# microsoft/SEAL

Measured on NVIDIA B200. Metric: CKKS multiply+relinearize ciphertexts/s, higher is better.
Workload: dtype u64

## Files before the change

### seal_b200/csrc/sb_api.cu

```cuda
#include "../../include/seal_b200.h"
#include "sb_engine.cuh"
#include <random>
#include <algorithm>
#include <cctype>
#include <cstdio>
#include <cstring>
#include <new>
#include <thread>

using namespace sb;

static thread_local std::string g_last_error;

struct sb200_context
{
    std::unique_ptr<Context> c;
};
struct sb200_public_key
{
    PublicKey k;
    ~sb200_public_key()
    {
        if (k.d_key && k.ctx)
        {
            cudaSetDevice(k.ctx->device);
            cudaFree(k.d_key);
        }
    }
};
struct sb200_secret_key
{
    SecretKey k;
    ~sb200_secret_key()
    {
        if (k.d_pow && k.ctx)
        {
            cudaSetDevice(k.ctx->device);
            cudaMemset(k.d_pow, 0, k.powers * k.ctx->k * k.ctx->n * sizeof(u64));
            cudaDeviceSynchronize();
        }
        cudaFree(k.d_pow);
    }
};
struct sb200_kswitch_key
{
    KSwitchKey k;
    ~sb200_kswitch_key()
    {
        if (k.ctx)
            cudaSetDevice(k.ctx->device);
        cudaFree(k.d_key);
        cudaFree(k.d_key32);
    }
};

#define SB_TRY try {
#define SB_CATCH                                   \
    }                                              \
    catch (const std::invalid_argument &e)         \
    {                                              \
        g_last_error = e.what();                   \
        return SB200_E_INVALID_ARG;                \
    }                                              \
    catch (const std::out_of_range &e)             \
    {                                              \
        g_last_error = e.what();                   \
        return SB200_E_OUT_OF_RANGE;               \
    }                                              \
    catch (const std::logic_error &e)              \
    {                                              \
        g_last_error = e.what();                   \
        return SB200_E_LOGIC;                      \
    }                                              \
    catch (const std::bad_alloc &e)                \
    {                                              \
        g_last_error = e.what();                   \
        return SB200_E_NOMEM;                      \
    }                                              \
    catch (const std::exception &e)                \
    {                                              \
        g_last_error = e.what();                   \
        return SB200_E_CUDA;                       \
    }

#define SB_NEED(p)                                      \
    if (!(p))                                           \
    {                                                   \
        g_last_error = "null pointer: " #p;             \
        return SB200_E_POINTER;                         \
    }

extern "C" {

const char *sb200_last_error(void)
{
    return g_last_error.c_str();
}

int sb200_context_create(int scheme, size_t n, const uint64_t *coeff_modulus, size_t k, uint64_t plain_modulus, int device,
                         sb200_context **out)
{
    SB_NEED(coeff_modulus);
    SB_NEED(out);
    SB_TRY
    auto h = std::make_unique<sb200_context>();
    h->c = make_context(scheme, n, reinterpret_cast<const u64 *>(coeff_modulus), k, plain_modulus, device);
    *out = h.release();
    return SB200_OK;
    SB_CATCH
}

int sb200_context_destroy(sb200_context *ctx)
{
    SB_NEED(ctx);
    delete ctx;
    return SB200_OK;
}

int sb200_coeff_modulus_create(size_t n, const int *bit_sizes, size_t k, uint64_t *out)
{
    SB_NEED(bit_sizes);
    SB_NEED(out);
    SB_TRY
    if (n < 2 || (n & (n - 1)) || n > 131072)
        throw std::invalid_argument("poly_modulus_degree is invalid");
    for (size_t i = 0; i < k; i++)
        if (bit_sizes[i] < 2 || bit_sizes[i] > 60)
            throw std::invalid_argument("bit_sizes is invalid");
    auto v = sbh::coeff_modulus_create(n, std::vector<int>(bit_sizes, bit_sizes + k));
    for (size_t i = 0; i < k; i++)
        out[i] = v[i];
    return SB200_OK;
    SB_CATCH
}

int sb200_get_ntt_tables(const sb200_context *ctx, size_t i, uint64_t *root, uint64_t *rp_op, uint64_t *rp_quo, uint64_t *irp_op,
                         uint64_t *inv_n)
{
    SB_NEED(ctx);
    SB_TRY
    const Context &c = *ctx->c;
    if (i >= c.k)
        throw std::out_of_range("prime_index");
    const auto &t = c.tabs[i];
    if (root)
        *root = t.root;
    if (inv_n)
        *inv_n = t.inv_n.w;
    for (size_t j = 0; j < c.n; j++)
    {
        if (rp_op)
            rp_op[j] = t.root_powers[j].w;
        if (rp_quo)
            rp_quo[j] = t.root_powers[j].wq;
        if (irp_op)
            irp_op[j] = t.inv_root_powers[j].w;
    }
    return SB200_OK;
    SB_CATCH
}

int sb200_get_base_bsk(const sb200_context *ctx, size_t L, uint64_t *out, size_t capacity, size_t *count)
{
    SB_NEED(ctx);
    SB_NEED(out);
    SB_NEED(count);
    SB_TRY
    Context &c = *ctx->c;
    if (c.scheme != SB200_SCHEME_BFV)
        throw std::logic_error("BEHZ base exists for BFV contexts only");
    const auto &b = behz_host(c, L);
    if (b.nBsk > capacity)
        throw std::out_of_range("capacity");
    for (size_t i = 0; i < b.nBsk; i++)
        out[i] = b.Bsk[i];
    *count = b.nBsk;
    return SB200_OK;
    SB_CATCH
}

uint32_t sb200_galois_elt_from_step(const sb200_context *ctx, int step)
{
    if (!ctx)
        return 0;
    try
    {
        return sbh::galois_elt_from_step(ctx->c->n, step);
    }
    catch (const std::exception &e)
    {
        g_last_error = e.what();
        return 0;
    }
}

unsigned long long sb200_launch_count(const sb200_context *ctx)
{
    return ctx ? ctx->c->stats.launches : 0;
}

size_t sb200_device_bytes(const sb200_context *ctx)
{
    return ctx ? ctx->c->table_bytes + ctx->c->scratch_bytes + ctx->c->aux_bytes : 0;
}

// ... 1488 lines not shown
```

### seal_b200/csrc/sb_engine.cuh

```cuda
#pragma once
#include "sb_host.hpp"
#include "sb_ntt.cuh"
#include "sb_ksint.cuh"
#include "sb_wire.hpp"
#include <array>
#include <map>
#include <memory>
#include <mutex>
#include <string>
#include <vector>

namespace sb
{
    struct CudaError : std::runtime_error
    {
        using std::runtime_error::runtime_error;
    };
    void cuda_check(cudaError_t e, const char *what);

    struct BehzDev;

    struct SecretKey
    {
        struct Context *ctx = nullptr;
        u64 *d_pow = nullptr;
        size_t powers = 0;
    };

    struct PublicKey
    {
        struct Context *ctx = nullptr;
        u64 *d_key = nullptr;
    };

    struct KSwitchKey
    {
        struct Context *ctx = nullptr;
        u64 *d_key = nullptr;
        uint32_t *d_key32 = nullptr;
        size_t digits = 0;
    };

    struct IoArena
    {
        bool ready = false;
        cudaStream_t s_in = nullptr, s_comp = nullptr, s_out = nullptr;
        cudaEvent_t ev_in[2] = {}, ev_comp[2] = {}, ev_out[2] = {};
        u64 *buf[2][3] = {};
        size_t cap[2][3] = {};
        struct Lane
        {
            void *pin[2] = {};
            size_t cap = 0;
            cudaEvent_t ev[2] = {}, order = nullptr;
            cudaStream_t st = nullptr;
            std::mutex mu;
        } lane[2];
    };

    struct Context
    {
        int scheme = 0, device = 0, logn = 0;
        bool fast_q = true;
        size_t n = 0, k = 0;
        u64 t = 0;
        std::vector<u64> q;
        std::vector<sbh::PrimeTables> tabs;
        std::vector<u64> aux;
        std::vector<Tw *> d_fwd, d_inv;
        PrimeDev *d_primes = nullptr;
        size_t nprimes = 0;
        Tw *d_invq = nullptr;
        Tw *d_qmod = nullptr;
        u64 t_ratio = 0;
        std::vector<u64> inv_q_mod_t;
        struct DecryptLevel
        {
            void *d_consts = nullptr;
            u64 neg_inv_q_mod_t = 0, neg_inv_q_mod_g = 0, q_mod_t = 0;
        };
        std::map<size_t, DecryptLevel> decrypt_levels;
        int t_pid = -1;
        uint32_t *d_batch_inv_map = nullptr;
        struct PlainLevel
        {
            Tw *d_delta = nullptr;
            u64 q_mod_t = 0;
        };
        std::map<size_t, PlainLevel> plain_levels;
        struct CkksEncoder
        {
            bool ready = false;
            void *d_roots = nullptr, *d_inv_roots = nullptr;
            uint32_t *d_map = nullptr;
            void *d_stat = nullptr;
        } ckks;
        struct CkksLevel
        {
            int total_bits = 0;
            u64 *d_big = nullptr;
            Tw *d_invp = nullptr;
        };
        std::map<size_t, CkksLevel> ckks_levels;
        u64 *d_t_mod_q = nullptr;
        u64 t_ratio_lo = 0, t_ratio_hi = 0;
        std::vector<std::array<u64, 4>> parms_ids;
        std::map<uint32_t, uint32_t *> galois_tables;
        std::map<size_t, std::shared_ptr<BehzDev>> behz;
        void *scratch = nullptr;
        int *d_flag = nullptr;
        void *aux_buf = nullptr;
        size_t aux_bytes = 0;
        size_t scratch_used = 0, aux_used = 0;
        size_t scratch_bytes = 0, table_bytes = 0, scratch_budget = size_t(8) << 30;
        size_t ks_chunk_max = 0;
        size_t host_stage_bytes = size_t(640) << 20;
        LaunchStats stats;
        KsInt ksint;
        int ks_algo = 1;
        size_t ks_min_digits = 6;
        bool ksint_on(size_t L) const { return ksint.ready && (ks_algo == 2 || (ks_algo == 1 && L >= ks_min_digits)); }
        IoArena io;
        std::mutex mu;
        cudaEvent_t order_event = nullptr;
        cudaStream_t order_stream = nullptr;
        bool order_valid = false;

        ~Context();
        void *ensure_scratch(size_t bytes);
        void *ensure_aux(size_t bytes);
        void wipe_scratch(cudaStream_t st);
        void wipe_aux(cudaStream_t st);
        const uint32_t *galois_table(uint32_t elt);
        size_t prime_id_aux(size_t aux_index) const { return k + aux_index; }
    };

    std::unique_ptr<Context> make_context(int scheme, size_t n, const u64 *moduli, size_t k, u64 t, int device);

    void op_ntt(Context &c, bool inverse, size_t L, size_t size, size_t batch, u64 *d, cudaStream_t st);
    void op_linear(Context &c, int mode, size_t L, size_t size, size_t batch, const u64 *a, const u64 *b, u64 *out, cudaStream_t st);
    void op_multiply_plain(Context &c, size_t L, size_t size, size_t batch, const u64 *a, const u64 *plain, u64 *out, cudaStream_t st);
    void secret_key_create(Context &c, const u64 *h_sk, SecretKey &out);
    void op_decrypt(Context &c, SecretKey &sk, size_t L, size_t size, size_t batch, const u64 *ct, const u64 *h_cf, u64 *plain, cudaStream_t st);
    void op_batch_encode(Context &c, size_t batch, const u64 *values, u64 *plain, cudaStream_t st);
    void op_batch_decode(Context &c, size_t batch, const u64 *plain, u64 *values, cudaStream_t st);
    void op_plain_to_ntt(Context &c, size_t L, size_t batch, const u64 *plain, const u64 *h_cf, u64 *out, cudaStream_t st);
    void op_multiply_plain_coeff(Context &c, size_t L, size_t size, size_t batch, bool ct_ntt, const u64 *ct, const u64 *plain, u64 *out,
                                 cudaStream_t st);
    void op_add_plain_coeff(Context &c, size_t L, size_t size, size_t batch, bool subtract, const u64 *ct, const u64 *plain, const u64 *h_cf,
                            u64 *out, cudaStream_t st);
    void op_ckks_multiply(Context &c, size_t L, size_t batch, const u64 *a, const u64 *b, u64 *out3, cudaStream_t st);
    void op_bfv_multiply(Context &c, size_t L, size_t batch, const u64 *a, const u64 *b, u64 *out3, cudaStream_t st);
    void op_ckks_multiply(Context &c, size_t L, size_t s1, size_t s2, size_t batch, const u64 *a, const u64 *b, u64 *out, cudaStream_t st);
    void op_bfv_multiply(Context &c, size_t L, size_t s1, size_t s2, size_t batch, const u64 *a, const u64 *b, u64 *out, cudaStream_t st);
    void check_sizes(size_t s1, size_t s2);
    void launch_tensor_general(Context &c, const u64 *xa, long long xa_bs, const u64 *xb, long long xb_bs, u64 *out, const int *pid_tab,
                               size_t nb, size_t s1, size_t s2, size_t B, cudaStream_t st);
    void op_relinearize(Context &c, size_t L, size_t batch, const u64 *in3, const KSwitchKey &key, u64 *out2, cudaStream_t st);
    void op_multiply_relinearize(Context &c, size_t L, size_t batch, const u64 *a, const u64 *b, const KSwitchKey &key,
                                 u64 *out2, cudaStream_t st);
    void op_rescale(Context &c, size_t L, size_t polys, const u64 *in, u64 *out, cudaStream_t st);
    void op_mod_switch(Context &c, size_t L, size_t polys, const u64 *in, u64 *out, cudaStream_t st);
    void op_relinearize_sized(Context &c, size_t L, size_t size, size_t batch, const u64 *in, const KSwitchKey &key, u64 *out, cudaStream_t st);
    void op_apply_galois(Context &c, size_t L, size_t batch, const u64 *in2, uint32_t elt, const KSwitchKey &key, u64 *out2,
                         cudaStream_t st);
    size_t keyswitch_chunk(const Context &c, size_t L, size_t batch, bool fused);
    double selftest_rate(Context &c, int kind, cudaStream_t st);
    void op_expand_seeded(Context &c, size_t L, size_t B, const u64 *h_seeds, const long long *h_dst_off, u64 *d_out, cudaStream_t st);
    void op_encrypt_zero_symmetric(Context &c, const SecretKey &sk, size_t L, size_t B, const u64 *h_boot_seeds, bool save_seed, u64 *d_out,
                                   u64 *h_public_seeds, cudaStream_t st);
    void public_key_create(Context &c, const u64 *h_pk, PublicKey &out);
    void op_encrypt_zero_asymmetric(Context &c, const PublicKey &pk, size_t L, size_t B, const u64 *h_seeds, u64 *d_out, cudaStream_t st);
    void op_ckks_encode(Context &c, size_t L, size_t B, const double *values, size_t count, bool is_complex, double scale, u64 *plain,
                        cudaStream_t st);
    void op_ckks_decode(Context &c, size_t L, size_t B, const u64 *plain, double scale, double *values, cudaStream_t st);
    const sbh::BehzLevel &behz_host(Context &c, size_t L);
    bool op_residues_in_range(Context &c, size_t L, size_t rows, const u64 *d, cudaStream_t st);
}
```

### seal_b200/csrc/sb_ksint.cu

```cuda
#include "sb_engine.cuh"
#include "sb_ksint.cuh"
#include <algorithm>
#include <cstdlib>

namespace sb
{
    struct P32
    {
        uint32_t p, p2, np;
    };
    __device__ __forceinline__ P32 make_p32(uint32_t p) { return P32{ p, 2 * p, 0u - p }; }
    __device__ __forceinline__ uint32_t minsub(uint32_t x, uint32_t m) { return min(x, x - m); }
    __device__ __forceinline__ uint32_t mul32_lazy(uint32_t y, uint2 w, uint32_t np) { return y * w.x + __umulhi(y, w.y) * np; }
    __device__ __forceinline__ void ct32(uint32_t &x, uint32_t &y, uint2 w, const P32 &P)
    {
        const uint32_t u = minsub(x, P.p2), t = mul32_lazy(y, w, P.np);
        x = u + t;
        y = u - t + P.p2;
    }
    __device__ __forceinline__ void gs32(uint32_t &x, uint32_t &y, uint2 w, const P32 &P)
    {
        const uint32_t u = x + y, v = x - y + P.p2;
        x = minsub(u, P.p2);
        y = mul32_lazy(v, w, P.np);
// ... 332 lines not shown
        asm volatile("cp.async.wait_group %0;" ::"n"(D - 2) : "memory");
        fetch(dA, kA, 0);
        int J = 0;
#pragma unroll 1
        for (; J + 2 <= L; J += 2)
        {
            issue();
            asm volatile("cp.async.wait_group %0;" ::"n"(D - 2) : "memory");
            fetch(dB, kB, J + 1);
            macs(dA, kA);
            issue();
            asm volatile("cp.async.wait_group %0;" ::"n"(D - 2) : "memory");
            fetch(dA, kA, J + 2);
            macs(dB, kB);
        }
        if (J < L)
            macs(dA, kA);
        asm volatile("cp.async.wait_group 0;" ::: "memory");
        const P32 P = make_p32(prm.p[t]);
        const uint2 red = prm.red[t];
        const uint32_t mu = prm.mu[t];
#pragma unroll
        for (int i = 0; i < TB; i++)
        {
            if (b0 + i < B)
            {
                uint32_t *o = Acc + ((((static_cast<size_t>(b0 + i) * 2 + c) * (L + 1) + i0) * prm.S + t) << LOGN) + x;
#pragma unroll
                for (int r = 0; r < TC; r++)
                    if (i0 + r <= L)
                        o[(static_cast<size_t>(r) * prm.S) << LOGN] = minsub(reduce64(acc[i][r], red, mu, P), P.p2);
            }
        }
    }
    constexpr int kMacRingBytes = kMacStages * kMacTB * 512 * 4;
    template <int LOGN>
    __global__ void __launch_bounds__(512, 1) ks32_mac_tile(const uint32_t *__restrict__ Dh, const uint32_t *__restrict__ key32, uint32_t *__restrict__ Acc,
                                                             KsIntParams prm, int L, int k, int digits, int B, int Bpad)
    {
        constexpr int TB = kMacTB, TC = kMacTC, D = kMacStages;
        extern __shared__ __align__(16) uint32_t ks_tile[];
        const int warp = threadIdx.x >> 5, lane = threadIdx.x & 31;
        const int ntile = (L + TC) / TC, ny = (2 * ntile + 3) / 4;
        const int yg = blockIdx.x % ny, xt = blockIdx.x / ny, t = blockIdx.z;
        const int x = (xt << 5) + lane;
        const uint32_t *kbase = key32 + ((static_cast<size_t>(t) * digits * 2 * k) << LOGN) + x;
        const size_t kstep = static_cast<size_t>(2 * k) << LOGN;
        for (int rho = warp; rho < L * 32; rho += 16)
        {
            const int J = rho >> 5, tr = rho & 31;
            const int task = min(yg * 4 + (tr >> 3), 2 * ntile - 1), c = task / ntile, i0 = (task - c * ntile) * TC;
            cp_async4(ks_tile + ((((J << 3) + (tr >> 2)) << 5) + lane) * 4 + (tr & 3),
                      kbase + J * kstep + (static_cast<size_t>(c * k + i0 + (tr & 7)) << LOGN));
        }
        asm volatile("cp.async.commit_group;\n\tcp.async.wait_group 0;" ::: "memory");
        __syncthreads();
        const int bsub = warp & 3, icsub = warp >> 2;
        const int task = yg * 4 + icsub;
        if (task >= 2 * ntile)
            return;
        const int c = task / ntile, i0 = (task - c * ntile) * TC;
        const uint32_t *ktile = ks_tile + (((icsub * 2) << 5) + lane) * 4;
        uint32_t *ring = ks_tile + L * 1024 + threadIdx.x * 4;
        const P32 P = make_p32(prm.p[t]);
        const uint2 red = prm.red[t];
        const uint32_t mu = prm.mu[t];
        const size_t dstep = static_cast<size_t>(Bpad) << LOGN;
        for (int b0 = bsub * TB; b0 < B; b0 += 4 * TB)
        {
            const uint32_t *dp = Dh + ((static_cast<size_t>(t) * L * Bpad + b0) << LOGN) + x;
            u64 acc[TB][TC];
#pragma unroll
            for (int i = 0; i < TB; i++)
#pragma unroll
                for (int r = 0; r < TC; r++)
                    acc[i][r] = 0;
            auto issue_quad = [&](int stage, int J) {
#pragma unroll
                for (int h = 0; h < 4; h++)
                    if (J + h < L)
                    {
                        uint32_t *dst = ring + (stage + h) * (TB * 512);
#pragma unroll
                        for (int i = 0; i < TB; i++)
                            cp_async4(dst + i, dp + (i << LOGN));
                        dp += dstep;
                    }
                asm volatile("cp.async.commit_group;" ::: "memory");
            };
            static_assert(TB == 4 && TC == 8 && D == 8, "operand fetches are 16-byte reads; the ring holds two groups of four digits");
            auto pair_step = [&](int stage, const uint32_t *kt, bool both) {
                uint32_t d0[TB], k0[TC], d1[TB], k1[TC];
                const uint32_t *src = ring + stage * (TB * 512);
                const uint4 da = *reinterpret_cast<const uint4 *>(src), db = *reinterpret_cast<const uint4 *>(src + TB * 512);
                const uint4 ka = *reinterpret_cast<const uint4 *>(kt), kb = *reinterpret_cast<const uint4 *>(kt + 128);
                const uint4 kc = *reinterpret_cast<const uint4 *>(kt + 1024), kd = *reinterpret_cast<const uint4 *>(kt + 1024 + 128);
                d0[0] = da.x, d0[1] = da.y, d0[2] = da.z, d0[3] = da.w, d1[0] = db.x, d1[1] = db.y, d1[2] = db.z, d1[3] = db.w;
                k0[0] = ka.x, k0[1] = ka.y, k0[2] = ka.z, k0[3] = ka.w, k0[4] = kb.x, k0[5] = kb.y, k0[6] = kb.z, k0[7] = kb.w;
                k1[0] = kc.x, k1[1] = kc.y, k1[2] = kc.z, k1[3] = kc.w, k1[4] = kd.x, k1[5] = kd.y, k1[6] = kd.z, k1[7] = kd.w;
                if (both)
                {
#pragma unroll
                    for (int i = 0; i < TB; i++)
#pragma unroll
                        for (int r = 0; r < TC; r++)
                        {
                            asm("mad.wide.u32 %0, %1, %2, %0;" : "+l"(acc[i][r]) : "r"(d0[i]), "r"(k0[r]));
                            asm("mad.wide.u32 %0, %1, %2, %0;" : "+l"(acc[i][r]) : "r"(d1[i]), "r"(k1[r]));
                        }
                }
                else
                {
#pragma unroll
                    for (int i = 0; i < TB; i++)
#pragma unroll
                        for (int r = 0; r < TC; r++)
                            asm("mad.wide.u32 %0, %1, %2, %0;" : "+l"(acc[i][r]) : "r"(d0[i]), "r"(k0[r]));
                }
            };
            issue_quad(0, 0);
            const uint32_t *kt = ktile;
#pragma unroll 1
            for (int J0 = 0; J0 < L; J0 += D)
            {
#pragma unroll
                for (int u = 0; u < D; u += 4)
                {
                    const int J = J0 + u;
                    if (J >= L)
                        break;
                    issue_quad((u + 4) & (D - 1), J + 4);
                    asm volatile("cp.async.wait_group 1;" ::: "memory");
                    pair_step(u, kt, J + 1 < L);
                    if (J + 2 < L)
                        pair_step(u + 2, kt + 2048, J + 3 < L);
                    kt += 4096;
                }
            }
            asm volatile("cp.async.wait_group 0;" ::: "memory");
#pragma unroll
            for (int i = 0; i < TB; i++)
            {
                if (b0 + i < B)
                {
                    uint32_t *o = Acc + ((((static_cast<size_t>(b0 + i) * 2 + c) * (L + 1) + i0) * prm.S + t) << LOGN) + x;
#pragma unroll
                    for (int r = 0; r < TC; r++)
                        if (i0 + r <= L)
                            o[(static_cast<size_t>(r) * prm.S) << LOGN] = minsub(reduce64(acc[i][r], red, mu, P), P.p2);
                }
            }
        }
    }
    template <int LOGN>
    static void launch_mac(const KsIntScratch &s, const uint32_t *key32, const KsInt &d, int L, int k, int digits, int B, int nbt, int n,
                           cudaStream_t st)
    {
        const int ntile = (L + kMacTC) / kMacTC, ny = (2 * ntile + 3) / 4;
        const size_t tile_smem = static_cast<size_t>(L) * 4096 + kMacRingBytes;
        if (d.mac_tile && tile_smem <= 227 * 1024 && B >= 16)
        {
            cuda_check(cudaFuncSetAttribute(ks32_mac_tile<LOGN>, cudaFuncAttributeMaxDynamicSharedMemorySize, static_cast<int>(tile_smem)), "smem attr");
            dim3 grid(static_cast<unsigned>(ny) * static_cast<unsigned>(n / 32), 1, static_cast<unsigned>(d.prm.S));
            ks32_mac_tile<LOGN><<<grid, 512, tile_smem, st>>>(s.Dh, key32, s.Acc, d.prm, L, k, digits, B, nbt * kMacTB);
            return;
        }
        cuda_check(cudaFuncSetAttribute(ks32_mac<LOGN>, cudaFuncAttributeMaxDynamicSharedMemorySize, kMacSmem), "smem attr");
        dim3 grid(static_cast<unsigned>(nbt) * static_cast<unsigned>(ny) * static_cast<unsigned>(n / 32), 1, static_cast<unsigned>(d.prm.S));
        ks32_mac<LOGN><<<grid, 128, kMacSmem, st>>>(s.Dh, key32, s.Acc, d.prm, L, k, digits, B, nbt);
    }

    struct CrtArgs
    {
        const uint32_t *Acc;
        const u64 *punct, *neg;
        const PrimeDev *primes;
        const Tw *inv_top;
        const u64 *half_mod;
        const Tw *qtop_mod;
        u64 t = 0, t_ratio = 0;
        Tw inv_top_mod_t = { 0, 0 };
        u64 *R;
        u64 *out;
        long long o_bs, o_ps;
        BaseSrc base;
        int L, k;
        long long total;
    };
    template <int MODE, int LOGN, bool FUSE>
    __global__ void __launch_bounds__(FUSE ? 128 : 256) ks32_crt_kernel(CrtArgs A, KsIntParams prm, const uint2 *__restrict__ tw_outer)
    {
        constexpr int R = LOGN - 12, E = FUSE ? (1 << R) : 1;
        const int S = prm.S, L = A.L, k = A.k;
        int bc, j;
        if (FUSE)
            bc = blockIdx.x >> 5, j = ((blockIdx.x & 31) << 7) + threadIdx.x;
        else
        {
            const long long e = static_cast<long long>(blockIdx.x) * blockDim.x + threadIdx.x;
            if (e >= A.total)
                return;
            bc = static_cast<int>(e >> LOGN), j = static_cast<int>(e & ((1 << LOGN) - 1));
        }
        const int b = bc >> 1, c = bc & 1;
        const uint32_t *src = A.Acc + ((static_cast<size_t>(bc) * (L + 1) * S) << LOGN) + j;
        constexpr int PF = FUSE ? 1 : kKsMaxS;
        uint32_t nxt[PF];
        auto prefetch = [&]() {
            if (!FUSE)
            {
#pragma unroll
                for (int t = 0; t < kKsMaxS; t++)
                    if (t < S)
                        nxt[t] = src[static_cast<size_t>(t) << LOGN];
            }
        };
        prefetch();
        uint32_t nrow[FUSE ? E : 1];
        int rows_left = FUSE ? (L + 1) * S : 0;
        auto fetch_row = [&]() {
            if (FUSE)
            {
                if (rows_left > 0)
                {
#pragma unroll
                    for (int e = 0; e < E; e++)
                        nrow[e] = src[e << 12];
                }
                src += size_t(1) << LOGN;
                rows_left--;
            }
        };
        fetch_row();
        auto reconstruct = [&](int ki, const PrimeDev &Q, u64(&val)[E], bool more) {
            u64 a0[E], a1[E], f[E];
#pragma unroll
            for (int e = 0; e < E; e++)
                a0[e] = a1[e] = f[e] = 0;
            const u64 *punct = A.punct + ki * S;
            uint32_t cur[PF];
            if (!FUSE)
            {
#pragma unroll
                for (int t = 0; t < kKsMaxS; t++)
                    cur[t] = nxt[t];
                src += static_cast<size_t>(S) << LOGN;
                if (more)
                    prefetch();
            }
#pragma unroll
            for (int t = 0; t < kKsMaxS; t++)
            {
                if (t >= S)
                    break;
                const P32 P = make_p32(prm.p[t]);
                uint32_t a[E];
                if (FUSE)
                {
#pragma unroll
                    for (int e = 0; e < E; e++)
                        a[e] = nrow[e];
                    fetch_row();
                    const uint2 *tw = tw_outer + (t << R);
                    radix_inv<R>(a, [&](int lvl, int g) { return __ldg(tw + (1 << lvl) + g); }, P);
                }
                else
                    a[0] = cur[t];
                const uint2 c1 = prm.c1[t];
                const uint32_t c2 = prm.c2[t], ip = prm.inv60[t];
                const u64 C = __ldg(punct + t);
                const uint32_t C0 = static_cast<uint32_t>(C), C1 = static_cast<uint32_t>(C >> 32);
#pragma unroll
                for (int e = 0; e < E; e++)
                {
                    const uint32_t y = minsub(minsub(a[e] * c1.x + c2 + __umulhi(a[e], c1.y) * P.np, P.p2), P.p);
                    asm("mad.wide.u32 %0, %1, %2, %0;" : "+l"(a0[e]) : "r"(y), "r"(C0));
                    asm("mad.wide.u32 %0, %1, %2, %0;" : "+l"(a1[e]) : "r"(y), "r"(C1));
                    asm("mad.wide.u32 %0, %1, %2, %0;" : "+l"(f[e]) : "r"(y), "r"(ip));
                }
            }
            const u64 *neg = A.neg + ki * S;
#pragma unroll
            for (int e = 0; e < E; e++)
            {
                const u64 ng = __ldg(neg + static_cast<int>(f[e] >> 60));
                u64 lo = a0[e] + (a1[e] << 32), hi = (a1[e] >> 32) + (lo < a0[e]);
                lo += ng;
                hi += (lo < ng);
                val[e] = barrett_wide(lo, hi, Q);
            }
        };
        const PrimeDev T = A.primes[k - 1];
        u64 U[E], K[MODE == 3 ? E : 1];
        reconstruct(k - 1, T, U, L > 0);
#pragma unroll
        for (int e = 0; e < E; e++)
        {
            if (MODE == 3)
            {
                const u64 r = barrett64(U[e], A.t, A.t_ratio);
                K[e] = mul_shoup(r ? A.t - r : 0, A.inv_top_mod_t, A.t);
            }
            else
                U[e] = csub(U[e] + (T.q >> 1), T.q);
        }
        for (int i = 0; i < L; i++)
        {
            const PrimeDev Q = A.primes[i];
            u64 a[E];
            reconstruct(i, Q, a, i + 1 < L);
// ... 69 lines not shown
            const u64 t = csub(csub(v, P.q2), P.q);
            out[b * o_bs + c * o_ps + (static_cast<long long>(i) << logn) + idx] = csub(t + base.get(b, c, i, idx, P.q), P.q);
        }
        __device__ __forceinline__ void store8(int row, int idx0, u64 (&a)[8], const PrimeDev &P) const
        {
            const int i = row % L, bc = row / L, b = bc >> 1, c = bc & 1;
            ulonglong2 *op_ = reinterpret_cast<ulonglong2 *>(out + b * o_bs + c * o_ps + (static_cast<long long>(i) << logn) + idx0);
            const bool has_base = base.present && !(c == 1 && base.c1_zero);
            const bool base_plain = has_base && base.s.plain();
            const ulonglong2 *bp = base_plain ? reinterpret_cast<const ulonglong2 *>(base.s.row(b, i) + c * base.pstride + idx0) : nullptr;
#pragma unroll
            for (int h = 0; h < 4; h++)
            {
                u64 r0 = csub(csub(a[2 * h], P.q2), P.q), r1 = csub(csub(a[2 * h + 1], P.q2), P.q);
                if (base_plain)
                {
                    const ulonglong2 bv = bp[h];
                    r0 = csub(r0 + bv.x, P.q), r1 = csub(r1 + bv.y, P.q);
                }
                else if (has_base)
                {
                    r0 = csub(r0 + base.get(b, c, i, idx0 + 2 * h, P.q), P.q);
                    r1 = csub(r1 + base.get(b, c, i, idx0 + 2 * h + 1, P.q), P.q);
                }
                op_[h] = make_ulonglong2(r0, r1);
            }
        }
    };

    template <class T>
    static T *upload(const std::vector<T> &v, size_t &bytes)
    {
        T *d = nullptr;
        cuda_check(cudaMalloc(reinterpret_cast<void **>(&d), std::max<size_t>(1, v.size()) * sizeof(T)), "cudaMalloc(ksint table)");
        cuda_check(cudaMemcpy(d, v.data(), v.size() * sizeof(T), cudaMemcpyHostToDevice), "upload ksint table");
        bytes += v.size() * sizeof(T);
        return d;
    }

    void ksint_init(Context &c)
    {
        c.ksint.ready = false;
        if (c.logn < 12 || c.k < 2)
            return;
        const sbh::KsIntHost h = sbh::build_ksint(c.n, c.q.data(), c.k);
        if (h.S == 0 || h.S > kKsMaxS)
            return;
        KsInt &d = c.ksint;
        d.prm.S = h.S, d.prm.r = h.r, d.prm.logn = c.logn;
        for (int t = 0; t < h.S; t++)
        {
            d.prm.p[t] = h.p[t], d.prm.mu[t] = h.mu[t], d.prm.c2[t] = h.c2[t];
            d.prm.inv60[t] = static_cast<uint32_t>((u64(1) << 60) / h.p[t]);
            d.prm.red[t] = make_uint2(h.red[2 * t], h.red[2 * t + 1]);
            d.prm.c1[t] = make_uint2(h.c1[2 * t], h.c1[2 * t + 1]);
        }
        d.d_fwd_outer = reinterpret_cast<uint2 *>(upload(h.fwd_outer, c.table_bytes));
        d.d_inv_outer = reinterpret_cast<uint2 *>(upload(h.inv_outer, c.table_bytes));
        d.d_fwd_local = reinterpret_cast<uint2 *>(upload(h.fwd_local, c.table_bytes));
        d.d_inv_local = reinterpret_cast<uint2 *>(upload(h.inv_local, c.table_bytes));
        d.d_punct = upload(h.punct_mod_q, c.table_bytes);
        d.d_neg = upload(h.neg_mod_q, c.table_bytes);
        {
            std::vector<u64> hm(c.k);
            for (size_t i = 0; i < c.k; i++)
                hm[i] = (c.q[c.k - 1] >> 1) % c.q[i];
            d.d_half_mod = upload(hm, c.table_bytes);
        }
        cuda_check(cudaFuncSetAttribute(ks32_fwd_local, cudaFuncAttributeMaxDynamicSharedMemorySize, kKsLocalSmem), "smem attr");
        cuda_check(cudaFuncSetAttribute(ks32_inv_local, cudaFuncAttributeMaxDynamicSharedMemorySize, kKsLocalSmem), "smem attr");
        if (const char *e = std::getenv("SB200_KS_FUSE_CRT"))
            d.fuse_crt = std::atoi(e) != 0;
        if (const char *e = std::getenv("SB200_KS_MAC_TILE"))
            d.mac_tile = std::atoi(e) != 0;
        d.ready = true;
    }
    void ksint_free(Context &c)
    {
        KsInt &d = c.ksint;
        cudaFree(d.d_fwd_outer), cudaFree(d.d_inv_outer), cudaFree(d.d_fwd_local), cudaFree(d.d_inv_local), cudaFree(d.d_punct), cudaFree(d.d_neg), cudaFree(d.d_half_mod);
        d = KsInt{};
    }

    size_t ksint_bytes_per_ct(const Context &c, size_t L)
    {
        const size_t S = c.ksint.prm.S;
        return c.n * (std::max(S * L * 4, 2 * L * 8) + 2 * (L + 1) * S * 4);
    }
    size_t ksint_bytes_fixed(const Context &c, size_t L) { return c.n * c.ksint.prm.S * L * 4 * (kMacTB - 1); }
    KsIntScratch ksint_carve(const Context &c, size_t L, size_t B, void *base)
    {
        const size_t S = c.ksint.prm.S, Bpad = (B + kMacTB - 1) / kMacTB * kMacTB;
        KsIntScratch s;
        unsigned char *p = static_cast<unsigned char *>(base);
        s.Dh = reinterpret_cast<uint32_t *>(p);
        s.R = reinterpret_cast<u64 *>(p);
        p += c.n * std::max(S * L * 4 * Bpad, 2 * L * 8 * B);
        s.Acc = reinterpret_cast<uint32_t *>(p);
        return s;
    }

    template <bool PLAIN>
    static void launch_fwd_outer(Context &c, Src dsrc, int L, int rows, uint32_t *Dh, RowMap map, cudaStream_t st)
    {
        const KsInt &d = c.ksint;
        const unsigned grid = static_cast<unsigned>(rows) * 16u;
        switch (d.prm.r)
        {
        case 0: ks32_fwd_outer<0, PLAIN><<<grid, 256, 0, st>>>(dsrc, L, c.d_primes, d.prm, d.d_fwd_outer, Dh, map); break;
        case 1: ks32_fwd_outer<1, PLAIN><<<grid, 256, 0, st>>>(dsrc, L, c.d_primes, d.prm, d.d_fwd_outer, Dh, map); break;
        case 2: ks32_fwd_outer<2, PLAIN><<<grid, 256, 0, st>>>(dsrc, L, c.d_primes, d.prm, d.d_fwd_outer, Dh, map); break;
        case 3: ks32_fwd_outer<3, PLAIN><<<grid, 256, 0, st>>>(dsrc, L, c.d_primes, d.prm, d.d_fwd_outer, Dh, map); break;
        case 4: ks32_fwd_outer<4, PLAIN><<<grid, 256, 0, st>>>(dsrc, L, c.d_primes, d.prm, d.d_fwd_outer, Dh, map); break;
        case 5: ks32_fwd_outer<5, PLAIN><<<grid, 256, 0, st>>>(dsrc, L, c.d_primes, d.prm, d.d_fwd_outer, Dh, map); break;
        default: throw std::logic_error("unsupported transform size");
        }
    }

    static void ksint_forward(Context &c, Src dsrc, int L, int rows, uint32_t *Dh, RowMap map, cudaStream_t st)
    {
        const KsInt &d = c.ksint;
        const double n = static_cast<double>(c.n), S = d.prm.S;
        const bool plain = dsrc.perm == nullptr && dsrc.ginv == 0;
        c.stats.begin("ks32_fwd_outer", 0, rows * n * (8.0 + 4.0 * S), st, 0, 0);
        c.stats.work32(0.5 * rows * n * S * d.prm.r, 0);
        plain ? launch_fwd_outer<true>(c, dsrc, L, rows, Dh, map, st) : launch_fwd_outer<false>(c, dsrc, L, rows, Dh, map, st);
        c.stats.end(st);
        cuda_check(cudaGetLastError(), "ks32_fwd_outer");
        dim3 grid(static_cast<unsigned>((map.rows_out + kRowsPerCta - 1) / kRowsPerCta), static_cast<unsigned>(d.prm.S << d.prm.r));
        c.stats.begin("ks32_fwd_local", 0, rows * n * 8.0 * S, st, 0, 0);
        c.stats.work32(0.5 * rows * n * S * 12, 0);
        ks32_fwd_local<<<grid, 256, kKsLocalSmem, st>>>(Dh, map.rows_out, 1, map.rows_out, d.prm, d.d_fwd_local);
        c.stats.end(st);
        cuda_check(cudaGetLastError(), "ks32_fwd_local");
    }

    void ksint_prepare_key(Context &c, KSwitchKey &key, cudaStream_t st)
    {
        if (!c.ksint.ready || key.d_key32)
            return;
        const size_t rows = key.digits * 2 * c.k, words = rows * c.n, S = c.ksint.prm.S;
        cuda_check(cudaMalloc(reinterpret_cast<void **>(&key.d_key32), (S * words + 8 * c.n) * sizeof(uint32_t)), "cudaMalloc(key, auxiliary primes)");
        cuda_check(cudaMemsetAsync(key.d_key32 + S * words, 0, 8 * c.n * sizeof(uint32_t), st), "memset");
        u64 *tmp = nullptr;
        cuda_check(cudaMalloc(reinterpret_cast<void **>(&tmp), words * sizeof(u64)), "cudaMalloc(key staging)");
        const bool prof = c.stats.profiling;
        c.stats.profiling = false;
        try
        {
            cuda_check(cudaMemcpyAsync(tmp, key.d_key, words * sizeof(u64), cudaMemcpyDeviceToDevice, st), "key copy");
            op_ntt(c, true, c.k, 2, key.digits, tmp, st);
            ksint_forward(c, Src{ tmp, 0, nullptr, 0, c.logn }, static_cast<int>(rows), static_cast<int>(rows), key.d_key32,
                          RowMap{ 2, static_cast<int>(c.k), static_cast<int>(rows) }, st);
            cuda_check(cudaStreamSynchronize(st), "synchronize");
        }
        catch (...)
        {
            c.stats.profiling = prof;
            cudaFree(tmp);
            throw;
        }
        c.stats.profiling = prof;
        cuda_check(cudaFree(tmp), "cudaFree(key staging)");
    }

    template <int R>
    static void launch_inv_outer_r(uint32_t *data, unsigned grid, const KsInt &d, cudaStream_t st)
    {
        ks32_inv_outer<R><<<grid, 256, 0, st>>>(data, d.prm, d.d_inv_outer);
    }

    static void launch_inverse(Context &c, uint32_t *data, int arows, cudaStream_t st, bool outer = true);

    void ksint_core(Context &c, size_t L, size_t B, const KsIntScratch &s, Src dsrc, const KSwitchKey &key, BaseSrc base, u64 *out,
                    long long o_bs, cudaStream_t st)
    {
        const KsInt &d = c.ksint;
        if (!d.ready || !key.d_key32)
            throw std::logic_error("integer key-switching path is not initialised");
        const int Li = static_cast<int>(L), ki = static_cast<int>(c.k), Bi = static_cast<int>(B), S = d.prm.S;
        const double n = static_cast<double>(c.n);
        const int rows = Bi * Li, nic = 2 * (Li + 1), arows = Bi * nic;
        const int nbt = (Bi + kMacTB - 1) / kMacTB, Bpad = nbt * kMacTB;
        ksint_forward(c, dsrc, Li, rows, s.Dh, RowMap{ 1, Bpad, Li * Bpad }, st);
        {
            c.stats.begin("ks32_mac", 0, 4.0 * n * S * (static_cast<double>(Li) * 2 * (Li + 1) + rows + arows), st);
            c.stats.work32(0, static_cast<double>(arows) * Li * S * n);
            const int dg = static_cast<int>(key.digits), ni = static_cast<int>(c.n);
            switch (c.logn)
            {
            case 12: launch_mac<12>(s, key.d_key32, d, Li, ki, dg, Bi, nbt, ni, st); break;
            case 13: launch_mac<13>(s, key.d_key32, d, Li, ki, dg, Bi, nbt, ni, st); break;
            case 14: launch_mac<14>(s, key.d_key32, d, Li, ki, dg, Bi, nbt, ni, st); break;
            case 15: launch_mac<15>(s, key.d_key32, d, Li, ki, dg, Bi, nbt, ni, st); break;
            case 16: launch_mac<16>(s, key.d_key32, d, Li, ki, dg, Bi, nbt, ni, st); break;
            case 17: launch_mac<17>(s, key.d_key32, d, Li, ki, dg, Bi, nbt, ni, st); break;
            default: throw std::logic_error("unsupported transform size");
            }
            c.stats.end(st);
            cuda_check(cudaGetLastError(), "ks32_mac");
        }
        const bool fuse_crt = d.fuse_crt && d.prm.r >= 1 && d.prm.r <= 4;
        launch_inverse(c, s.Acc, arows, st, !fuse_crt);
        const long long o_ps = static_cast<long long>(L) * c.n;
        if (!o_bs)
            o_bs = 2 * o_ps;
        {
            CrtArgs A{};
            A.Acc = s.Acc, A.punct = d.d_punct, A.neg = d.d_neg, A.primes = c.d_primes;
            A.inv_top = c.d_invq + (c.k - 1) * c.k;
            A.half_mod = d.d_half_mod;
            A.R = s.R, A.out = out, A.o_bs = o_bs, A.o_ps = o_ps, A.base = base, A.L = Li, A.k = ki;
            A.total = static_cast<long long>(B) * 2 * c.n;
            c.stats.begin("ks32_crt", 0, n * B * 2 * (4.0 * S * (L + 1) + 8.0 * L), st);
            if (fuse_crt)
                c.stats.work32(0.5 * arows * S * n * d.prm.r, 0);
            if (c.scheme == 3)
            {
                A.qtop_mod = c.d_qmod + (c.k - 1) * c.k;
                A.t = c.t, A.t_ratio = c.t_ratio;
                A.inv_top_mod_t = Tw{ c.inv_q_mod_t[c.k - 1], sbh::shoup(c.inv_q_mod_t[c.k - 1], c.t) };
                launch_crt<3>(A, d, fuse_crt, B, c.logn, st);
            }
            else if (c.scheme == 1)
                launch_crt<1>(A, d, fuse_crt, B, c.logn, st);
            else
                launch_crt<0>(A, d, fuse_crt, B, c.logn, st);
            c.stats.end(st);
            cuda_check(cudaGetLastError(), "ks32_crt_kernel");
        }
        if (c.scheme != 1)
        {
            OpAddBaseFwd op{ s.R, out, o_bs, o_ps, base, c.logn, Li };
            cuda_check(launch_ntt_fwd(op, static_cast<int>(B * 2 * L), c.logn, c.d_primes, st, c.stats, "ks_result_ntt", -1, c.fast_q), "ks result ntt");
        }
    }

    static void launch_inverse(Context &c, uint32_t *data, int arows, cudaStream_t st, bool outer)
    {
        const KsInt &d = c.ksint;
        const int S = d.prm.S;
        const double n = static_cast<double>(c.n);
        dim3 grid(static_cast<unsigned>((arows + kRowsPerCta - 1) / kRowsPerCta), static_cast<unsigned>(S << d.prm.r));
        c.stats.begin("ks32_inv_local", 0, 8.0 * arows * S * n, st);
        c.stats.work32(0.5 * arows * S * n * 12, 0);
        ks32_inv_local<<<grid, 256, kKsLocalSmem, st>>>(data, arows, S, 1, d.prm, d.d_inv_local);
        c.stats.end(st);
        cuda_check(cudaGetLastError(), "ks32_inv_local");
        if (d.prm.r > 0 && outer)
        {
            const unsigned g1 = static_cast<unsigned>(arows) * S * 16u;
            c.stats.begin("ks32_inv_outer", 0, 8.0 * arows * S * n, st);
            c.stats.work32(0.5 * arows * S * n * d.prm.r, 0);
            switch (d.prm.r)
            {
            case 1: launch_inv_outer_r<1>(data, g1, d, st); break;
            case 2: launch_inv_outer_r<2>(data, g1, d, st); break;
            case 3: launch_inv_outer_r<3>(data, g1, d, st); break;
            case 4: launch_inv_outer_r<4>(data, g1, d, st); break;
            case 5: launch_inv_outer_r<5>(data, g1, d, st); break;
            default: throw std::logic_error("unsupported transform size");
            }
            c.stats.end(st);
            cuda_check(cudaGetLastError(), "ks32_inv_outer");
        }
    }

    void ksint_selftest_transform(Context &c, bool inverse, const u64 *h_rows, size_t rows, uint32_t *h_io)
    {
        if (!c.ksint.ready)
            throw std::logic_error("integer key-switching path is not available for this context");
        const size_t S = c.ksint.prm.S, out_bytes = S * rows * c.n * sizeof(uint32_t), in_bytes = rows * c.n * sizeof(u64);
        unsigned char *base = static_cast<unsigned char *>(c.ensure_scratch(out_bytes + in_bytes));
        uint32_t *d32 = reinterpret_cast<uint32_t *>(base);
        if (inverse)
        {
            cuda_check(cudaMemcpy(d32, h_io, out_bytes, cudaMemcpyHostToDevice), "upload");
            launch_inverse(c, d32, static_cast<int>(rows), nullptr);
        }
        else
        {
            u64 *d64 = reinterpret_cast<u64 *>(base + out_bytes);
            cuda_check(cudaMemcpy(d64, h_rows, in_bytes, cudaMemcpyHostToDevice), "upload");
            ksint_forward(c, Src{ d64, 0, nullptr, 0, c.logn }, static_cast<int>(rows), static_cast<int>(rows), d32,
                          RowMap{ 0, 0, static_cast<int>(rows) }, nullptr);
        }
        cuda_check(cudaMemcpy(h_io, d32, out_bytes, cudaMemcpyDeviceToHost), "download");
    }

    template <int KIND>
    __global__ void __launch_bounds__(256, 4) ks32_selftest_bfly(uint32_t *d, uint32_t p, int rounds)
    {
        __shared__ uint2 ts[256];
        const P32 P = make_p32(p);
        {
            const uint32_t w = (threadIdx.x * 2654435761u + 12345u) % p;
            ts[threadIdx.x] = make_uint2(w, static_cast<uint32_t>((static_cast<u64>(w) << 32) / p));
        }
        __syncthreads();
        uint32_t a[16];
#pragma unroll
        for (int j = 0; j < 16; j++)
            a[j] = d[(static_cast<size_t>(blockIdx.x) * 16 + j) * 256 + threadIdx.x] % p;
        const int lane = threadIdx.x & 31;
        for (int r = 0; r < rounds; r++)
        {
            const uint2 *t = ts + ((r * 7 + lane) & 127);
            auto tw = [&](int lvl, int g) { return t[(1 << lvl) - 1 + g]; };
            if (KIND == 0)
                radix_fwd<4>(a, tw, P);
            else
                radix_inv<4>(a, tw, P);
        }
#pragma unroll
        for (int j = 0; j < 16; j++)
            d[(static_cast<size_t>(blockIdx.x) * 16 + j) * 256 + threadIdx.x] = a[j];
    }
    template <int THREADS, int MINB, bool PAIRED>
    __global__ void __launch_bounds__(THREADS, MINB) ks32_selftest_mac(uint32_t *d, int rounds)
    {
        uint32_t dv[4], kv[8];
        u64 acc[4][8];
#pragma unroll
        for (int i = 0; i < 4; i++)
            dv[i] = d[(static_cast<size_t>(blockIdx.x) * 12 + i) * THREADS + threadIdx.x] >> 3;
#pragma unroll
        for (int r = 0; r < 8; r++)
            kv[r] = d[(static_cast<size_t>(blockIdx.x) * 12 + 4 + r) * THREADS + threadIdx.x] >> 3;
#pragma unroll
        for (int i = 0; i < 4; i++)
#pragma unroll
            for (int r = 0; r < 8; r++)
                acc[i][r] = 0;
        for (int q = 0; q < rounds; q++)
        {
            uint32_t d0[4], k0[8], d1[4], k1[8];
#pragma unroll
            for (int i = 0; i < 4; i++)
                d0[i] = dv[i] + q, d1[i] = dv[i] ^ q;
#pragma unroll
            for (int r = 0; r < 8; r++)
                k0[r] = kv[r] ^ q, k1[r] = kv[r] + q;
#pragma unroll
            for (int i = 0; i < 4; i++)
#pragma unroll
                for (int r = 0; r < 8; r++)
                {
                    asm("mad.wide.u32 %0, %1, %2, %0;" : "+l"(acc[i][r]) : "r"(d0[i]), "r"(k0[r]));
                    if (PAIRED)
// ... 67 lines not shown
```

Measured before the change: 2860.

## Run key-switch MAC on int8 tensor cores with byte-plane decomposed keys

Adds a tensor-core MAC kernel for the integer key-switching path. It splits the 32-bit digit and key residues into byte planes and multiplies them with u8 mma.sync, then recombines the partial sums with shifts and a modular reduction. The key is re-laid out once at key creation into a tensor-core-friendly layout and used by default when k<=32. The aim is to replace scalar 32-bit modular MACs with much higher-throughput int8 MMA work. The cost is extra key memory and about sixteen times more partial products, plus correctness risk if the accumulators overflow.

```diff
diff --git a/seal_b200/csrc/sb_api.cu b/seal_b200/csrc/sb_api.cu
--- a/seal_b200/csrc/sb_api.cu
+++ b/seal_b200/csrc/sb_api.cu
@@ -51,6 +51,7 @@
             cudaSetDevice(k.ctx->device);
         cudaFree(k.d_key);
         cudaFree(k.d_key32);
+        cudaFree(k.d_keytc);
     }
 };
 
diff --git a/seal_b200/csrc/sb_engine.cuh b/seal_b200/csrc/sb_engine.cuh
--- a/seal_b200/csrc/sb_engine.cuh
+++ b/seal_b200/csrc/sb_engine.cuh
@@ -38,6 +38,7 @@
         struct Context *ctx = nullptr;
         u64 *d_key = nullptr;
         uint32_t *d_key32 = nullptr;
+        uint32_t *d_keytc = nullptr;
         size_t digits = 0;
     };
 
diff --git a/seal_b200/csrc/sb_ksint.cu b/seal_b200/csrc/sb_ksint.cu
--- a/seal_b200/csrc/sb_ksint.cu
+++ b/seal_b200/csrc/sb_ksint.cu
@@ -508,10 +508,161 @@
             }
         }
     }
+    constexpr int kTcX = 16, kTcB = 16, kTcStage = 168 * kTcB;
+    constexpr int kTcKeyWords = 4 * 64 * 8;
+    constexpr int kTcSmem = (kTcX * kTcKeyWords + 2 * 32 * kTcB * kTcX + 2 * kTcStage) * 4;
+    static_assert(kTcSmem <= 227 * 1024, "shared memory of ks32_mac_tc");
+    __device__ __forceinline__ int tc_pos(int b, int q, int x) { return (8 * b + (q ^ (b & 4))) ^ ((x & 7) | ((x & 8) << 1)); }
+    __device__ __forceinline__ void cp_async16(uint32_t *dst_smem, const uint32_t *src, bool valid)
+    {
+        asm volatile("cp.async.cg.shared.global [%0], [%1], 16, %2;" ::"r"(smem_u32(dst_smem)), "l"(src), "r"(valid ? 16 : 0) : "memory");
+    }
+    __device__ __forceinline__ void mma_u8(uint32_t (&d)[4], const uint32_t (&a)[4], uint2 b)
+    {
+        asm("mma.sync.aligned.m16n8k32.row.col.s32.u8.u8.s32 {%0,%1,%2,%3}, {%4,%5,%6,%7}, {%8,%9}, {%0,%1,%2,%3};"
+                     : "+r"(d[0]), "+r"(d[1]), "+r"(d[2]), "+r"(d[3])
+                     : "r"(a[0]), "r"(a[1]), "r"(a[2]), "r"(a[3]), "r"(b.x), "r"(b.y));
+    }
+    __global__ void __launch_bounds__(512, 1) ks32_mac_tc(const uint32_t *__restrict__ Dh, const uint32_t *__restrict__ keytc, uint32_t *__restrict__ Acc,
+                                                          KsIntParams prm, int L, int B, int Bpad)
+    {
+        extern __shared__ __align__(16) uint32_t tc_smem[];
+        uint32_t *ks = tc_smem, *raw = ks + kTcX * kTcKeyWords, *planes = raw + 32 * kTcB * kTcX, *stage = planes + 32 * kTcB * kTcX;
+        const int tid = threadIdx.x, warp = tid >> 5, lane = tid & 31, t = blockIdx.z, x0 = blockIdx.x * kTcX, logn = prm.logn;
+        {
+            const uint32_t *src = keytc + ((static_cast<size_t>(t) << logn) + x0) * kTcKeyWords;
+            for (int i = tid; i < kTcX * kTcKeyWords / 4; i += 512)
+                cp_async16(ks + 4 * i, src + 4 * i, true);
+        }
+        auto load_raw = [&](int b0) {
+#pragma unroll
+            for (int h = 0; h < 4; h++)
+            {
+                const int i = tid + 512 * h, J = i >> 6, b = (i >> 2) & 15, xc = i & 3;
+                const bool valid = J < L && b0 + b < B;
+                const uint32_t *src = Dh + ((static_cast<size_t>(t * L + (valid ? J : 0)) * Bpad + (valid ? b0 + b : 0)) << logn) + x0 + 4 * xc;
+                cp_async16(raw + 4 * i, src, valid);
+            }
+            asm volatile("cp.async.commit_group;" ::: "memory");
+        };
+        load_raw(0);
+        asm volatile("cp.async.wait_group 0;" ::: "memory");
+        __syncthreads();
+        const P32 P = make_p32(prm.p[t]);
+        const uint2 red = prm.red[t];
+        const uint32_t mu = prm.mu[t];
+        const int g = lane >> 2, tq = lane & 3, ntc = (L + 8) / 8;
+        const uint32_t *kx = ks + warp * kTcKeyWords + 2 * tq;
+        for (int b0 = 0; b0 < B; b0 += kTcB)
+        {
+            {
+                const int x = lane & 15, b = 2 * (warp & 7) + (lane >> 4);
+#pragma unroll
+                for (int qq = 0; qq < 4; qq++)
+                {
+                    const int q = (warp >> 3) * 4 + qq;
+                    const uint32_t *r = raw + (4 * q) * (kTcB * kTcX) + b * kTcX + x;
+                    const uint32_t w0 = r[0], w1 = r[kTcB * kTcX], w2 = r[2 * kTcB * kTcX], w3 = r[3 * kTcB * kTcX];
+                    const uint32_t t0 = __byte_perm(w0, w1, 0x5140), t1 = __byte_perm(w0, w1, 0x7362);
+                    const uint32_t t2 = __byte_perm(w2, w3, 0x5140), t3 = __byte_perm(w2, w3, 0x7362);
+                    uint32_t *p = planes + x * 512 + tc_pos(b, q, x);
+                    p[0] = __byte_perm(t0, t2, 0x5410);
+                    p[128] = __byte_perm(t0, t2, 0x7632);
+                    p[256] = __byte_perm(t1, t3, 0x5410);
+                    p[384] = __byte_perm(t1, t3, 0x7632);
+                }
+            }
+            __syncthreads();
+            if (b0 + kTcB < B)
+                load_raw(b0 + kTcB);
+            uint32_t A[4][4];
+            {
+                const uint32_t *p = planes + warp * 512;
+#pragma unroll
+                for (int a = 0; a < 4; a++)
+                {
+                    A[a][0] = p[a * 128 + tc_pos(g, tq, warp)];
+                    A[a][1] = p[a * 128 + tc_pos(g + 8, tq, warp)];
+                    A[a][2] = p[a * 128 + tc_pos(g, tq + 4, warp)];
+                    A[a][3] = p[a * 128 + tc_pos(g + 8, tq + 4, warp)];
+                }
+            }
+            int j = 0;
+            for (int c = 0; c < 2; c++)
+                for (int it = 0; it < ntc; it++, j++)
+                {
+                    uint32_t C[7][4] = {};
+                    const uint32_t *kb = kx + (c * 32 + it * 8 + g) * 8;
+#pragma unroll
+                    for (int pb = 0; pb < 4; pb++)
+                    {
+                        const uint2 bf = *reinterpret_cast<const uint2 *>(kb + pb * 512);
+#pragma unroll
+                        for (int a = 0; a < 4; a++)
+                            mma_u8(C[a + pb], A[a], bf);
+                    }
+                    uint32_t *sg = stage + (j & 1) * kTcStage;
+#pragma unroll
+                    for (int h = 0; h < 2; h++)
+                    {
+                        uint32_t r[2];
+#pragma unroll
+                        for (int e = 0; e < 2; e++)
+                        {
+                            const int v = 2 * h + e;
+                            const u64 lo = static_cast<u64>(C[0][v]) + (static_cast<u64>(C[1][v]) << 8) + (static_cast<u64>(C[2][v]) << 16) +
+                                           (static_cast<u64>(C[3][v]) << 24);
+                            const u64 hi = static_cast<u64>(C[4][v]) + (static_cast<u64>(C[5][v]) << 8) + (static_cast<u64>(C[6][v]) << 16);
+                            r[e] = minsub(reduce64(lo + (hi << 32), red, mu, P), P.p2);
+                        }
+                        *reinterpret_cast<uint2 *>(sg + 168 * (g + 8 * h) + 8 * warp + 8 * (warp >> 2) + 2 * tq) = make_uint2(r[0], r[1]);
+                    }
+                    __syncthreads();
+                    {
+                        const int b = tid >> 5, o = (tid >> 2) & 7, xc = tid & 3, I = it * 8 + o;
+                        if (b0 + b < B && I <= L)
+                        {
+                            const uint32_t *s = sg + 168 * b + 40 * xc + o;
+                            uint32_t *dst = Acc + (((static_cast<size_t>((b0 + b) * 2 + c) * (L + 1) + I) * prm.S + t) << logn) + x0 + 4 * xc;
+                            *reinterpret_cast<uint4 *>(dst) = make_uint4(s[0], s[8], s[16], s[24]);
+                        }
+                    }
+                }
+            asm volatile("cp.async.wait_group 0;" ::: "memory");
+            __syncthreads();
+        }
+    }
+    __global__ void ks32_key_tc(const uint32_t *__restrict__ key32, uint32_t *__restrict__ keytc, int k, int digits, int logn, size_t total)
+    {
+        const size_t i = static_cast<size_t>(blockIdx.x) * blockDim.x + threadIdx.x;
+        if (i >= total)
+            return;
+        const int x = static_cast<int>(i & ((size_t(1) << logn) - 1));
+        const size_t r = i >> logn;
+        const int q = static_cast<int>(r & 7), o = static_cast<int>((r >> 3) & 63), t = static_cast<int>(r >> 9);
+        const int c = o >> 5, I = o & 31;
+        uint32_t w[4];
+#pragma unroll
+        for (int j = 0; j < 4; j++)
+        {
+            const int J = 4 * q + j;
+            w[j] = (J < digits && I < k) ? key32[((((static_cast<size_t>(t) * digits + J) * 2 + c) * k + I) << logn) + x] : 0;
+        }
+        uint32_t *dst = keytc + ((static_cast<size_t>(t) << logn) + x) * kTcKeyWords + o * 8 + 2 * (q & 3) + (q >> 2);
+        for (int a = 0; a < 4; a++)
+            dst[a * 512] = ((w[0] >> (8 * a)) & 255) | (((w[1] >> (8 * a)) & 255) << 8) | (((w[2] >> (8 * a)) & 255) << 16) | (((w[3] >> (8 * a)) & 255) << 24);
+    }
     template <int LOGN>
-    static void launch_mac(const KsIntScratch &s, const uint32_t *key32, const KsInt &d, int L, int k, int digits, int B, int nbt, int n,
-                           cudaStream_t st)
-    {
+    static void launch_mac(const KsIntScratch &s, const uint32_t *key32, const uint32_t *keytc, const KsInt &d, int L, int k, int digits, int B,
+                           int nbt, int n, cudaStream_t st)
+    {
+        if (keytc)
+        {
+            cuda_check(cudaFuncSetAttribute(ks32_mac_tc, cudaFuncAttributeMaxDynamicSharedMemorySize, kTcSmem), "smem attr");
+            ks32_mac_tc<<<dim3(static_cast<unsigned>(n / kTcX), 1, static_cast<unsigned>(d.prm.S)), 512, kTcSmem, st>>>(s.Dh, keytc, s.Acc, d.prm, L, B,
+                                                                                                                   nbt * kMacTB);
+            return;
+        }
         const int ntile = (L + kMacTC) / kMacTC, ny = (2 * ntile + 3) / 4;
         const size_t tile_smem = static_cast<size_t>(L) * 4096 + kMacRingBytes;
         if (d.mac_tile && tile_smem <= 227 * 1024 && B >= 16)
@@ -887,6 +1038,14 @@
             op_ntt(c, true, c.k, 2, key.digits, tmp, st);
             ksint_forward(c, Src{ tmp, 0, nullptr, 0, c.logn }, static_cast<int>(rows), static_cast<int>(rows), key.d_key32,
                           RowMap{ 2, static_cast<int>(c.k), static_cast<int>(rows) }, st);
+            if (c.k <= 32)
+            {
+                const size_t total = S * 64 * 8 * c.n;
+                cuda_check(cudaMalloc(reinterpret_cast<void **>(&key.d_keytc), S * c.n * kTcKeyWords * sizeof(uint32_t)), "cudaMalloc(key, tensor-core layout)");
+                ks32_key_tc<<<static_cast<unsigned>((total + 255) / 256), 256, 0, st>>>(key.d_key32, key.d_keytc, static_cast<int>(c.k),
+                                                                                       static_cast<int>(key.digits), c.logn, total);
+                cuda_check(cudaGetLastError(), "ks32_key_tc");
+            }
             cuda_check(cudaStreamSynchronize(st), "synchronize");
         }
         catch (...)
@@ -922,14 +1081,16 @@
             c.stats.begin("ks32_mac", 0, 4.0 * n * S * (static_cast<double>(Li) * 2 * (Li + 1) + rows + arows), st);
             c.stats.work32(0, static_cast<double>(arows) * Li * S * n);
             const int dg = static_cast<int>(key.digits), ni = static_cast<int>(c.n);
+            const char *tc_env = std::getenv("SB200_KS_MAC_TC");
+            const uint32_t *keytc = (!tc_env || std::atoi(tc_env) != 0) ? key.d_keytc : nullptr;
             switch (c.logn)
             {
-            case 12: launch_mac<12>(s, key.d_key32, d, Li, ki, dg, Bi, nbt, ni, st); break;
-            case 13: launch_mac<13>(s, key.d_key32, d, Li, ki, dg, Bi, nbt, ni, st); break;
-            case 14: launch_mac<14>(s, key.d_key32, d, Li, ki, dg, Bi, nbt, ni, st); break;
-            case 15: launch_mac<15>(s, key.d_key32, d, Li, ki, dg, Bi, nbt, ni, st); break;
-            case 16: launch_mac<16>(s, key.d_key32, d, Li, ki, dg, Bi, nbt, ni, st); break;
-            case 17: launch_mac<17>(s, key.d_key32, d, Li, ki, dg, Bi, nbt, ni, st); break;
+            case 12: launch_mac<12>(s, key.d_key32, keytc, d, Li, ki, dg, Bi, nbt, ni, st); break;
+            case 13: launch_mac<13>(s, key.d_key32, keytc, d, Li, ki, dg, Bi, nbt, ni, st); break;
+            case 14: launch_mac<14>(s, key.d_key32, keytc, d, Li, ki, dg, Bi, nbt, ni, st); break;
+            case 15: launch_mac<15>(s, key.d_key32, keytc, d, Li, ki, dg, Bi, nbt, ni, st); break;
+            case 16: launch_mac<16>(s, key.d_key32, keytc, d, Li, ki, dg, Bi, nbt, ni, st); break;
+            case 17: launch_mac<17>(s, key.d_key32, keytc, d, Li, ki, dg, Bi, nbt, ni, st); break;
             default: throw std::logic_error("unsupported transform size");
             }
             c.stats.end(st);
```

After: 3434, median of 6. +20.1%, better.
